# zama-ai/verifiable-fhe-paper

Hardware: AMD Instinct MI355X
Metric: vPBS proofs/sec at N=1024 (1/2/4/8 GPU); prover ms/proof vs CPU baseline (higher is better)
Workload: dtype u64; 1 GPU; N=1024 vPBS as IVC chain (BASELINE config 2; verified_pbs ivc_based_vpbs.rs:159-386) via vpbs_ivc_prove_pbs; step = 1 chained proof of the cyclic circuit (2^16 rows) per chain; chains_per_gpu=8, parallelism=replicas, witness=host

## Files before the change

bindings/rust/vpbs_sys.rs:

```rust
#![allow(non_camel_case_types, dead_code)]
use std::os::raw::{c_char, c_long, c_void};

pub const VPBS_POW_ANY: u64 = u64::MAX;
pub const VPBS_UNUSED_SELECTOR: u32 = 0xFFFF_FFFF;

#[repr(C)] pub struct VpbsCtx { _private: [u8; 0] }
#[repr(C)] pub struct VpbsBatch { _private: [u8; 0] }
#[repr(C)] pub struct VpbsWitnessPlan { _private: [u8; 0] }
#[repr(C)] pub struct VpbsWitnessState { _private: [u8; 0] }
#[repr(C)] pub struct VpbsWitnessDevice { _private: [u8; 0] }
#[repr(C)] pub struct VpbsWitnessChecker { _private: [u8; 0] }
#[repr(C)] pub struct VpbsProofVerifier { _private: [u8; 0] }
#[repr(C)] pub struct VpbsIvc { _private: [u8; 0] }
#[repr(C)] pub struct VpbsPbsVerifier { _private: [u8; 0] }
#[repr(C)] pub struct VpbsRingVerifier { _private: [u8; 0] }
#[repr(C)] pub struct VpbsBootstrapper { _private: [u8; 0] }
#[repr(C)] pub struct VpbsKeyring { _private: [u8; 0] }
#[repr(C)] pub struct VpbsPbsProver { _private: [u8; 0] }
#[repr(C)] pub struct VpbsRingProver { _private: [u8; 0] }
#[repr(C)] pub struct VpbsProgram { _private: [u8; 0] }

pub const VPBS_OK: i32 = 0;
pub const VPBS_ERR_INVALID: i32 = -1;
pub const VPBS_ERR_DEVICE: i32 = -2;
// ... 414 lines not shown
    pub fn vpbs_verify_step(in_: *const VpbsVerifyInputs, caps: *const u64, openings: *const u64, fri: *const u64) -> i32;
    pub fn vpbs_proof_verifier_create(ctx: *mut VpbsCtx, circuit: *const VpbsVerifyInputs, max_batch: usize, max_public_inputs: usize, out: *mut *mut VpbsProofVerifier, err: *mut c_char, err_len: usize) -> i32;
    pub fn vpbs_proof_verifier_run(v: *mut VpbsProofVerifier, bytes: *const u8, offsets: *const usize, count: usize, verdicts: *mut u8, reasons: *mut u8) -> c_long;
    pub fn vpbs_proof_verifier_free(v: *mut VpbsProofVerifier);
    pub fn vpbs_ivc_create(ctx: *mut VpbsCtx, cyclic: *const VpbsIvcCircuit, dummy: *const VpbsIvcCircuit, n: u32, k: u32, ggsw_len: usize, comm: *const VpbsComm, out: *mut *mut VpbsIvc, err: *mut c_char, err_len: usize) -> i32;
    pub fn vpbs_ivc_free(ivc: *mut VpbsIvc);
    pub fn vpbs_ivc_set_device_witness(ivc: *mut VpbsIvc, ell: u32, logb: u32, batch: u32, late_on_device: i32) -> i32;
    pub fn vpbs_ivc_set_check_witness(ivc: *mut VpbsIvc, on: i32) -> i32;
    pub fn vpbs_ivc_witness_checks(ivc: *const VpbsIvc, out: *mut u64) -> i32;
    pub fn vpbs_ivc_set_step_callback(ivc: *mut VpbsIvc, fn_: Option<VpbsIvcStepFn>, user: *mut c_void) -> i32;
    pub fn vpbs_ivc_last_error(ivc: *const VpbsIvc) -> *const c_char;
    pub fn vpbs_ivc_verifier_data(ivc: *const VpbsIvc, cyclic_vk: *mut u64, dummy_vk: *mut u64) -> i32;
    pub fn vpbs_ivc_prove_pbs(ivc: *mut VpbsIvc, testv: *const u64, ct: *const u64, bsk: *const u64, ksk: *const u64, n_lwe: u32, steps: u32, proof_out: *mut u8, capacity: usize, timing: *mut VpbsIvcTiming, err: *mut c_char, err_len: usize) -> c_long;
    pub fn vpbs_ivc_set_checkpoint(ivc: *mut VpbsIvc, every: u32, fn_: Option<VpbsIvcCheckpointFn>, user: *mut c_void) -> i32;
    pub fn vpbs_ivc_resume_pbs(ivc: *mut VpbsIvc, testv: *const u64, ct: *const u64, bsk: *const u64, ksk: *const u64, n_lwe: u32, checkpoint: *const u8, len: usize, steps: u32, proof_out: *mut u8, capacity: usize, timing: *mut VpbsIvcTiming, err: *mut c_char, err_len: usize) -> c_long;
    pub fn vpbs_verify_pbs(in_: *const VpbsVerifyPbsInputs, proof_bytes: *const u8, len: usize, why: *mut c_char, why_len: usize) -> i32;
    pub fn vpbs_verify_pbs_prefix(in_: *const VpbsVerifyPbsInputs, bytes: *const u8, len: usize, steps_done: *mut u32, why: *mut c_char, why_len: usize) -> i32;
    pub fn vpbs_pbs_reason_text(reason: i32) -> *const c_char;
    pub fn vpbs_pbs_key_hash(bsk: *const u64, ksk: *const u64, n_lwe: u32, ggsw_len: usize, out: *mut u64) -> i32;
    pub fn vpbs_pbs_verifier_create(ctx: *mut VpbsCtx, shape: *const VpbsVerifyPbsInputs, key_hash: *const u64, max_batch: usize, out: *mut *mut VpbsPbsVerifier, err: *mut c_char, err_len: usize) -> i32;
    pub fn vpbs_pbs_verifier_run(v: *mut VpbsPbsVerifier, bytes: *const u8, offsets: *const usize, count: usize, testv: *const u64, testv_per_proof: i32, ct: *const u64, out_ct: *const u64, verdicts: *mut u8, reasons: *mut u8, proof_reasons: *mut u8) -> c_long;
    pub fn vpbs_pbs_verifier_free(v: *mut VpbsPbsVerifier);
    pub fn vpbs_ring_verifier_create(ctx: *mut VpbsCtx, shape: *const VpbsVerifyPbsInputs, max_keys: u32, max_batch: usize, out: *mut *mut VpbsRingVerifier, err: *mut c_char, err_len: usize) -> i32;
    pub fn vpbs_ring_verifier_set_key(v: *mut VpbsRingVerifier, slot: u32, key_hash: *const u64) -> i32;
    pub fn vpbs_ring_verifier_clear_key(v: *mut VpbsRingVerifier, slot: u32) -> i32;
    pub fn vpbs_ring_verifier_count(v: *mut VpbsRingVerifier) -> c_long;
    pub fn vpbs_ring_verifier_run(v: *mut VpbsRingVerifier, bytes: *const u8, offsets: *const usize, count: usize, key_of: *const u32, testvs: *const u64, n_testv: usize, testv_of: *const u32, ct: *const u64, out_ct: *const u64, verdicts: *mut u8, reasons: *mut u8, proof_reasons: *mut u8, err: *mut c_char, err_len: usize) -> c_long;
    pub fn vpbs_ring_verifier_free(v: *mut VpbsRingVerifier);
    pub fn vpbs_k_poseidon_batch(ctx: *mut VpbsCtx, states: *mut u64, n: usize) -> i32;
    pub fn vpbs_k_hash_rows(ctx: *mut VpbsCtx, rows: *const u64, n: usize, len: u32, out: *mut u64) -> i32;
    pub fn vpbs_k_intt(ctx: *mut VpbsCtx, values: *const u64, ncols: u32, log_n: u32, coeffs_out: *mut u64) -> i32;
    pub fn vpbs_k_coset_lde(ctx: *mut VpbsCtx, coeffs: *const u64, ncols: u32, log_n: u32, rate_bits: u32, shift: u64, out: *mut u64) -> i32;
    pub fn vpbs_k_merkle_cap(ctx: *mut VpbsCtx, leaves: *const u64, n_leaves: usize, leaf_len: u32, cap_height: u32, cap_out: *mut u64) -> i32;
    pub fn vpbs_k_negacyclic_ntt(ctx: *mut VpbsCtx, data: *mut u64, batch: u32, log_n: u32, inverse: i32) -> i32;
    pub fn vpbs_k_poseidon_host(states: *mut u64, n: usize) -> i32;
    pub fn vpbs_k_clock_probe(ctx: *mut VpbsCtx, mhz_out: *mut f64) -> i32;
    pub fn vpbs_ntt_params(log_n: u32, roots: *mut u64, invroots: *mut u64, ninv: *mut u64) -> i32;
    pub fn vpbs_blind_rotate_step(ctx: *mut VpbsCtx, params: *const VpbsTfheParams, batch: u32, acc_in: *const u64, masks: *const u64, ggsw: *const u64, ggsw_per_instance: i32, first_step: i32, last_step: i32, acc_out: *mut u64, on_device: i32) -> i32;
    pub fn vpbs_pbs_accumulator_chain(ctx: *mut VpbsCtx, params: *const VpbsTfheParams, n: u32, acc_init: *const u64, lwe_ct: *const u64, bsk: *const u64, ksk: *const u64, accs_out: *mut u64) -> i32;
    pub fn vpbs_keygen(ctx: *mut VpbsCtx, params: *const VpbsKeygenParams, s_lwe: *mut u64, s_glwe: *mut u64, s_to: *mut u64, bsk: *mut u64, ksk: *mut u64, keys_on_device: i32) -> i32;
    pub fn vpbs_lwe_encrypt(params: *const VpbsKeygenParams, s_lwe: *const u64, message: u64, nonce: u64, ct: *mut u64) -> i32;
    pub fn vpbs_testv(log_n: u32, p: u32, testv: *mut u64, delta: *mut u64) -> i32;
    pub fn vpbs_glwe_decrypt(ctx: *mut VpbsCtx, log_n: u32, k: u32, s: *const u64, ct: *const u64, m_out: *mut u64) -> i32;
    pub fn vpbs_bootstrapper_create(ctx: *mut VpbsCtx, params: *const VpbsTfheParams, n_lwe: u32, bsk: *const u64, ksk: *const u64, keys_on_device: i32, max_batch: usize, out: *mut *mut VpbsBootstrapper, err: *mut c_char, err_len: usize) -> i32;
    pub fn vpbs_bootstrapper_run(b: *mut VpbsBootstrapper, cts: *const u64, count: usize, testv: *const u64, testv_per_ct: i32, out_ct: *mut u64, lwe_out: *mut u64, accs_out: *mut u64, on_device: i32) -> c_long;
    pub fn vpbs_bootstrapper_run_from(b: *mut VpbsBootstrapper, cts: *const u64, count: usize, start: *const u32, acc_in: *const u64, testv: *const u64, testv_per_ct: i32, out_ct: *mut u64, lwe_out: *mut u64, accs_out: *mut u64, on_device: i32) -> c_long;
    pub fn vpbs_bootstrapper_free(b: *mut VpbsBootstrapper);
    pub fn vpbs_lwe_extract(ctx: *mut VpbsCtx, log_n: u32, k: u32, n_lwe: u32, glwe: *const u64, count: usize, lwe_out: *mut u64, on_device: i32) -> i32;
    pub fn vpbs_lwe_decrypt(s_lwe: *const u64, ct: *const u64, n_lwe: u32, m_out: *mut u64) -> i32;
    pub fn vpbs_keyring_create(ctx: *mut VpbsCtx, params: *const VpbsTfheParams, n_lwe: u32, max_keys: usize, max_batch: usize, out: *mut *mut VpbsKeyring, err: *mut c_char, err_len: usize) -> i32;
    pub fn vpbs_keyring_add(ring: *mut VpbsKeyring, bsk: *const u64, ksk: *const u64, keys_on_device: i32, slot: *mut u32) -> i32;
    pub fn vpbs_keyring_remove(ring: *mut VpbsKeyring, slot: u32) -> i32;
    pub fn vpbs_keyring_count(ring: *mut VpbsKeyring) -> usize;
    pub fn vpbs_keyring_run(ring: *mut VpbsKeyring, cts: *const u64, count: usize, key_of: *const u32, testv: *const u64, testv_per_ct: i32, out_ct: *mut u64, lwe_out: *mut u64, accs_out: *mut u64, on_device: i32) -> c_long;
    pub fn vpbs_keyring_run_from(ring: *mut VpbsKeyring, cts: *const u64, count: usize, key_of: *const u32, start: *const u32, acc_in: *const u64, testv: *const u64, testv_per_ct: i32, out_ct: *mut u64, lwe_out: *mut u64, accs_out: *mut u64, on_device: i32) -> c_long;
    pub fn vpbs_keyring_free(ring: *mut VpbsKeyring);
    pub fn vpbs_lwe_encrypt_batch(ctx: *mut VpbsCtx, params: *const VpbsKeygenParams, s_lwe: *const u64, key_on_device: i32, messages: *const u64, count: usize, nonce0: u64, cts_out: *mut u64, on_device: i32) -> i32;
    pub fn vpbs_lut_testv(log_n: u32, p: u32, table: *const u64, delta: u64, testv: *mut u64) -> i32;
    pub fn vpbs_lwe_decode_batch(ctx: *mut VpbsCtx, s_lwe: *const u64, key_on_device: i32, cts: *const u64, count: usize, n_lwe: u32, delta: u64, modulus: u64, expected: *const u64, phase_out: *mut u64, msg_out: *mut u64, err_out: *mut u64, stats: *mut VpbsNoiseStats, on_device: i32) -> i32;
    pub fn vpbs_pbs_prover_create(device_ordinal: i32, cyclic: *const VpbsIvcCircuit, dummy: *const VpbsIvcCircuit, params: *const VpbsTfheParams, n_lwe: u32, bsk: *const u64, ksk: *const u64, keys_on_device: i32, chains: u32, witness_batch: u32, out: *mut *mut VpbsPbsProver, err: *mut c_char, err_len: usize) -> i32;
    pub fn vpbs_pbs_prover_run(p: *mut VpbsPbsProver, cts: *const u64, count: usize, testv: *const u64, testv_per_ct: i32, steps: u32, out_ct: *mut u64, lwe_out: *mut u64, proof_fn: Option<VpbsPbsProofFn>, user: *mut c_void, err: *mut c_char, err_len: usize) -> c_long;
    pub fn vpbs_pbs_prover_resume(p: *mut VpbsPbsProver, cts: *const u64, count: usize, testv: *const u64, testv_per_ct: i32, checkpoints: *const *const u8, lens: *const usize, steps: u32, out_ct: *mut u64, lwe_out: *mut u64, proof_fn: Option<VpbsPbsProofFn>, user: *mut c_void, err: *mut c_char, err_len: usize) -> c_long;
    pub fn vpbs_pbs_prover_key_hash(p: *const VpbsPbsProver, out: *mut u64) -> i32;
    pub fn vpbs_pbs_prover_verifier_data(p: *const VpbsPbsProver, cyclic_vk: *mut u64, dummy_vk: *mut u64) -> i32;
    pub fn vpbs_pbs_prover_set_check_witness(p: *mut VpbsPbsProver, on: i32) -> i32;
    pub fn vpbs_pbs_prover_witness_checks(p: *const VpbsPbsProver, out: *mut u64) -> i32;
// ... 44 lines not shown
```

include/vpbs_prover.h:

```cpp
#ifndef VPBS_PROVER_H
#define VPBS_PROVER_H
#include <stddef.h>
#include <stdint.h>

#ifdef __cplusplus
extern "C" {
#endif

typedef struct vpbs_ctx vpbs_ctx;
typedef struct vpbs_batch vpbs_batch;

typedef enum {
    VPBS_OK = 0,
    VPBS_ERR_INVALID = -1,
    VPBS_ERR_DEVICE = -2,
    VPBS_ERR_OOM = -3,
    VPBS_ERR_POW = -4,
    VPBS_ERR_PEER = -5,
    VPBS_ERR_WITNESS = -6
} vpbs_status;

#define VPBS_POW_ANY UINT64_MAX

int vpbs_ctx_create(int device_ordinal, unsigned log_n_max, unsigned rate_bits, unsigned cap_height, vpbs_ctx** out);
// ... 382 lines not shown
} vpbs_pbs_reason;
const char* vpbs_pbs_reason_text(int reason);
int vpbs_pbs_key_hash(const uint64_t* bsk , const uint64_t* ksk , unsigned n_lwe, size_t ggsw_len,
                      uint64_t out[4]);
typedef struct vpbs_pbs_verifier vpbs_pbs_verifier;
int vpbs_pbs_verifier_create(vpbs_ctx* ctx, const vpbs_verify_pbs_inputs* shape, const uint64_t key_hash[4], size_t max_batch,
                             vpbs_pbs_verifier** out, char* err, size_t err_len);
long vpbs_pbs_verifier_run(vpbs_pbs_verifier* v, const uint8_t* bytes, const size_t* offsets , size_t count,
                           const uint64_t* testv , int testv_per_proof, const uint64_t* ct ,
                           const uint64_t* out_ct , uint8_t* verdicts , uint8_t* reasons ,
                           uint8_t* proof_reasons );
void vpbs_pbs_verifier_free(vpbs_pbs_verifier* v);

typedef struct vpbs_ring_verifier vpbs_ring_verifier;
int vpbs_ring_verifier_create(vpbs_ctx* ctx, const vpbs_verify_pbs_inputs* shape, unsigned max_keys, size_t max_batch, vpbs_ring_verifier** out,
                              char* err, size_t err_len);
int vpbs_ring_verifier_set_key(vpbs_ring_verifier* v, unsigned slot, const uint64_t key_hash[4]);
int vpbs_ring_verifier_clear_key(vpbs_ring_verifier* v, unsigned slot);
long vpbs_ring_verifier_count(vpbs_ring_verifier* v);
long vpbs_ring_verifier_run(vpbs_ring_verifier* v, const uint8_t* bytes, const size_t* offsets , size_t count,
                            const uint32_t* key_of , const uint64_t* testvs , size_t n_testv,
                            const uint32_t* testv_of , const uint64_t* ct ,
                            const uint64_t* out_ct , uint8_t* verdicts , uint8_t* reasons ,
                            uint8_t* proof_reasons , char* err, size_t err_len);
void vpbs_ring_verifier_free(vpbs_ring_verifier* v);

int vpbs_k_poseidon_batch(vpbs_ctx* ctx, uint64_t* states , size_t n);
int vpbs_k_hash_rows(vpbs_ctx* ctx, const uint64_t* rows , size_t n, unsigned len, uint64_t* out );
int vpbs_k_intt(vpbs_ctx* ctx, const uint64_t* values, unsigned ncols, unsigned log_n, uint64_t* coeffs_out);
int vpbs_k_coset_lde(vpbs_ctx* ctx, const uint64_t* coeffs, unsigned ncols, unsigned log_n, unsigned rate_bits,
                     uint64_t shift, uint64_t* out);
int vpbs_k_merkle_cap(vpbs_ctx* ctx, const uint64_t* leaves, size_t n_leaves, unsigned leaf_len, unsigned cap_height,
                      uint64_t* cap_out);
int vpbs_k_negacyclic_ntt(vpbs_ctx* ctx, uint64_t* data, unsigned batch, unsigned log_n, int inverse);
int vpbs_k_poseidon_host(uint64_t* states, size_t n);
int vpbs_k_clock_probe(vpbs_ctx* ctx, double* mhz_out);
int vpbs_ntt_params(unsigned log_n, uint64_t* roots, uint64_t* invroots, uint64_t* ninv);

typedef struct {
    unsigned log_N;
    unsigned K;
    unsigned ELL;
    unsigned LOGB;
} vpbs_tfhe_params;
int vpbs_blind_rotate_step(vpbs_ctx* ctx, const vpbs_tfhe_params* params, unsigned batch, const uint64_t* acc_in,
                           const uint64_t* masks, const uint64_t* ggsw, int ggsw_per_instance, int first_step, int last_step,
                           uint64_t* acc_out, int on_device);

int vpbs_pbs_accumulator_chain(vpbs_ctx* ctx, const vpbs_tfhe_params* params, unsigned n, const uint64_t* acc_init,
                               const uint64_t* lwe_ct, const uint64_t* bsk, const uint64_t* ksk, uint64_t* accs_out);

typedef struct {
    unsigned log_N, K, ELL, LOGB;
    unsigned n_lwe;
    uint64_t seed;
    double sigma_glwe, sigma_lwe;
} vpbs_keygen_params;
int vpbs_keygen(vpbs_ctx* ctx, const vpbs_keygen_params* params, uint64_t* s_lwe, uint64_t* s_glwe, uint64_t* s_to, uint64_t* bsk,
                uint64_t* ksk, int keys_on_device);
int vpbs_lwe_encrypt(const vpbs_keygen_params* params, const uint64_t* s_lwe, uint64_t message, uint64_t nonce, uint64_t* ct);
int vpbs_testv(unsigned log_N, unsigned p, uint64_t* testv, uint64_t* delta);
int vpbs_glwe_decrypt(vpbs_ctx* ctx, unsigned log_N, unsigned K, const uint64_t* s, const uint64_t* ct, uint64_t* m_out);

typedef struct vpbs_bootstrapper vpbs_bootstrapper;
int vpbs_bootstrapper_create(vpbs_ctx* ctx, const vpbs_tfhe_params* params, unsigned n_lwe, const uint64_t* bsk, const uint64_t* ksk,
                             int keys_on_device, size_t max_batch, vpbs_bootstrapper** out, char* err, size_t err_len);
// ... 151 lines not shown
```

verifiable-fhe-paper_amd/api.py:

```python
import ctypes as C
import json
import math
import os
import subprocess
import weakref
from fractions import Fraction

import numpy as np

PKG_DIR = os.path.dirname(os.path.abspath(__file__))
LIB_PATH = os.path.join(PKG_DIR, "libvpbs_hip.so")
P = 0xFFFFFFFF00000001
POW_ANY = 0xFFFFFFFFFFFFFFFF
U64P = C.POINTER(C.c_uint64)
U32P = C.POINTER(C.c_uint32)


class VpbsError(RuntimeError):
    pass


ERR_WITNESS = -6


# ... 326 lines not shown
    "vpbs_ring_prover_keyring": (_vp, [_vp]),
    "vpbs_ring_prover_context": (_vp, [_vp]),
    "vpbs_ring_prover_run": (C.c_long, [_vp, U64P, _sz, _vp, U64P, _i, _ui, U64P, U64P, PBS_PROOF_FN, _vp, C.c_char_p, _sz]),
    "vpbs_ring_prover_resume": (C.c_long, [_vp, U64P, _sz, _vp, U64P, _i, _vp, _vp, _ui, U64P, U64P, PBS_PROOF_FN, _vp, C.c_char_p, _sz]),
    "vpbs_ring_prover_verifier_data": (_i, [_vp, U64P, U64P]),
    "vpbs_ring_prover_set_check_witness": (_i, [_vp, _i]),
    "vpbs_ring_prover_witness_checks": (_i, [_vp, U64P]),
    "vpbs_ring_prover_set_checkpoint": (_i, [_vp, _ui, PBS_CHECKPOINT_FN, _vp]),
    "vpbs_ring_prover_last_run": (_i, [_vp, C.POINTER(PbsRunStatsC)]),
    "vpbs_ring_prover_free": (None, [_vp]),
    "vpbs_program_create": (_i, [_vp, C.POINTER(ProgramDescC), C.POINTER(_vp), C.c_char_p, _sz]),
    "vpbs_program_levels": (C.c_long, [_vp, C.POINTER(_ui)]),
    "vpbs_program_run": (C.c_long, [_vp, _vp, _vp, _vp, _vp, _vp, _vp, _i]),
    "vpbs_program_run_batch": (C.c_long, [_vp, _vp, _vp, _sz, _vp, _vp, _vp, _vp, _vp, _i]),
    "vpbs_program_prove": (C.c_long, [_vp, _vp, U64P, U64P, _ui, U64P, U64P, PBS_PROOF_FN, _vp, C.c_char_p, _sz]),
    "vpbs_program_prove_batch": (C.c_long, [_vp, _vp, U64P, _sz, _vp, U64P, _ui, U64P, U64P, PBS_PROOF_FN, _vp, C.c_char_p, _sz]),
    "vpbs_program_verify": (C.c_long, [_vp, _vp, U64P, U64P, U64P, C.POINTER(C.c_uint8), C.POINTER(_sz), C.POINTER(C.c_uint8),
                                       C.POINTER(C.c_uint8), C.POINTER(C.c_uint8)]),
    "vpbs_program_verify_batch": (C.c_long, [_vp, _vp, U64P, _sz, _vp, U64P, U64P, C.POINTER(C.c_uint8), C.POINTER(_sz), C.POINTER(C.c_uint8),
                                             C.POINTER(C.c_uint8), C.POINTER(C.c_uint8), C.c_char_p, _sz]),
    "vpbs_program_free": (None, [_vp]),
    "vpbs_program_create_multi": (_i, [_vp, C.POINTER(ProgramDescC), C.POINTER(_ui), C.POINTER(_ui), C.POINTER(_vp), C.c_char_p, _sz]),
    "vpbs_program_wires": (C.c_long, [_vp, C.POINTER(_ui)]),
    "vpbs_lwe_snap": (_i, [_vp, _ui, _ui, _vp, _sz, _vp, _i]),
    "vpbs_lwe_extract_at": (_i, [_vp, _ui, _ui, _ui, _vp, _sz, _vp, _vp, _sz, _vp, _i]),
    "vpbs_lut_testv_multi": (_i, [_ui, _ui, _ui, U64P, _u64, U64P]),
    "vpbs_lwe_extract": (_i, [_vp, _ui, _ui, _ui, _vp, _sz, _vp, _i]),
    "vpbs_lwe_decrypt": (_i, [U64P, U64P, _ui, U64P]),
    "vpbs_lwe_encrypt_batch": (_i, [_vp, C.POINTER(KeygenParamsC), _vp, _i, _vp, _sz, _u64, _vp, _i]),
    "vpbs_lut_testv": (_i, [_ui, _ui, U64P, _u64, U64P]),
    "vpbs_lwe_decode_batch": (_i, [_vp, _vp, _i, _vp, _sz, _ui, _u64, _u64, _vp, _vp, _vp, _vp, C.POINTER(NoiseStatsC), _i]),
    "vpbs_k_poseidon_batch": (_i, [_vp, U64P, _sz]),
    "vpbs_k_hash_rows": (_i, [_vp, U64P, _sz, _ui, U64P]),
    "vpbs_k_intt": (_i, [_vp, U64P, _ui, _ui, U64P]),
    "vpbs_k_coset_lde": (_i, [_vp, U64P, _ui, _ui, _ui, _u64, U64P]),
    "vpbs_k_merkle_cap": (_i, [_vp, U64P, _sz, _ui, _ui, U64P]),
    "vpbs_k_negacyclic_ntt": (_i, [_vp, U64P, _ui, _ui, _i]),
    "vpbs_ntt_params": (_i, [_ui, U64P, U64P, U64P]),
    "vpbs_timing_enable": (_i, [_vp, _i]),
    "vpbs_timing_report": (_i, [_vp, C.c_char_p, _sz]),
    "vpbs_timing_shader_clock": (_i, [_vp, C.POINTER(C.c_double), C.POINTER(_ui)]),
}

INTERNAL_SIGNATURES = {
    "vpbs_test_ivc_preset_matrix": (_i, [_sz, _sz, _sz, _sz, _ui, _ui, _ui, U64P, U64P, U64P, U64P, U64P, U64P, U64P, U64P]),
    "vpbs_test_pbs_prover_preset_matrix": (_i, [_vp, U64P, U64P, _ui, _ui, U64P]),
    "vpbs_test_pbs_prover_preset_words": (_sz, [_vp]),
    "vpbs_test_pbs_prover_dummy_proof": (_i, [_vp, U64P]),
}

_lib = None


def build_library(force=False):
    args = ["make", "-C", os.path.join(PKG_DIR, "csrc"), "-j4"]
    if force:
        subprocess.check_call(args + ["clean"], stdout=subprocess.DEVNULL)
    subprocess.check_call(args, stdout=subprocess.DEVNULL)
    return LIB_PATH


def lib():
    global _lib
    if _lib is None:
        if not os.path.exists(LIB_PATH):
            raise VpbsError("libvpbs_hip.so is missing: run __graft_entry__.build() (make -C verifiable-fhe-paper_amd/csrc). "
# ... 2475 lines not shown
        self._check(lib().vpbs_k_clock_probe(self.h, C.byref(out)))
        return out.value

    def upload_bg(self, d_dst, host, words):
        if lib().vpbs_device_upload_bg(self.h, C.c_void_p(int(d_dst)), C.c_void_p(int(host)), int(words)):
            raise VpbsError("vpbs_device_upload_bg failed")

    def upload_rows(self, d_dst, host, n_cols, n, row_lo, row_hi):
        self._check(lib().vpbs_device_upload_rows(self.h, C.c_void_p(int(d_dst)), C.c_void_p(int(host)), n_cols, n, row_lo, row_hi))

    def scatter(self, d_dst, d_positions, host_values, count, d_stage):
        self._check(lib().vpbs_device_scatter(self.h, C.c_void_p(int(d_dst)), C.c_void_p(int(d_positions)), C.c_void_p(int(host_values)), count,
                                              C.c_void_p(int(d_stage))))

    def glwe_decrypt(self, s, ct):
        ct = _u64(ct)
        K, N = ct.shape
        s = np.ascontiguousarray(_u64(s)[:K - 1])
        out = np.zeros(N, np.uint64)
        self._check(lib().vpbs_glwe_decrypt(self.h, N.bit_length() - 1, K, _ptr(s), _ptr(ct), _ptr(out)))
        return out

    def poseidon_batch(self, states):
        s = _u64(states).copy()
        self._check(lib().vpbs_k_poseidon_batch(self.h, _ptr(s), s.shape[0]))
        return s

    def hash_rows(self, rows):
        r = _u64(rows)
        out = np.zeros((r.shape[0], 4), np.uint64)
        self._check(lib().vpbs_k_hash_rows(self.h, _ptr(r), r.shape[0], r.shape[1], _ptr(out)))
        return out

    def intt(self, values):
        v = _u64(values)
        out = np.zeros_like(v)
        self._check(lib().vpbs_k_intt(self.h, _ptr(v), v.shape[0], v.shape[1].bit_length() - 1, _ptr(out)))
        return out

    def coset_lde(self, coeffs, rate_bits=3, shift=7):
        c = _u64(coeffs)
        out = np.zeros((c.shape[0], c.shape[1] << rate_bits), np.uint64)
        self._check(lib().vpbs_k_coset_lde(self.h, _ptr(c), c.shape[0], c.shape[1].bit_length() - 1, rate_bits, shift, _ptr(out)))
        return out

    def merkle_cap(self, leaves, cap_height):
        l = _u64(leaves)
        out = np.zeros((1 << cap_height, 4), np.uint64)
        self._check(lib().vpbs_k_merkle_cap(self.h, _ptr(l), l.shape[0], l.shape[1], cap_height, _ptr(out)))
        return out

    def negacyclic_ntt(self, data, inverse=False):
        d = _u64(data).copy()
        self._check(lib().vpbs_k_negacyclic_ntt(self.h, _ptr(d), d.shape[0], d.shape[1].bit_length() - 1, 1 if inverse else 0))
        return d

    def timing_enable(self, on=1):
        self._check(lib().vpbs_timing_enable(self.h, int(on)))

    def timing_report(self):
        buf = C.create_string_buffer(8192)
        self._check(lib().vpbs_timing_report(self.h, buf, 8192))
        return json.loads(buf.value.decode())
```

verifiable-fhe-paper_amd/csrc/api.hip:

```cpp
#include <atomic>
#include <sys/prctl.h>
#include <time.h>
#include <chrono>
#include <condition_variable>
#include <cstdlib>
#include <cstring>
#include <memory>
#include <mutex>
#include <unordered_map>

#include "context.h"
#include "poseidon.h"
#include "host/poseidon_x8.h"

using vpbs::DeviceError;
using vpbs::u64;

void* vpbs_ctx::alloc_bytes(size_t bytes) {
    if (bytes == 0) bytes = 8;
    bytes = (bytes + 255) & ~(size_t)255;
    auto it = free_blocks.find(bytes);
    if (it != free_blocks.end()) {
        void* p = it->second;
        free_blocks.erase(it);
// ... 848 lines not shown
        u64* d_out = c->alloc_words(a.record_words);
        auto* d_args = static_cast<vpbs::OpenArgs*>(c->alloc_bytes(sizeof a));
        VPBS_HIP(hipMemcpyAsync(d_args, &a, sizeof a, hipMemcpyHostToDevice, c->stream));
        vpbs::launch_open_queries(c->stream, d_args, 1, 1, d_out);
        std::vector<u64> rec(a.record_words);
        VPBS_HIP(hipMemcpyAsync(rec.data(), d_out, sizeof(u64) * a.record_words, hipMemcpyDeviceToHost, c->stream));
        VPBS_HIP(vpbs::stream_sync(c->stream));
        std::memcpy(leaf_out, rec.data(), sizeof(u64) * b->ncols);
        std::memcpy(siblings_out, rec.data() + b->ncols, sizeof(u64) * 4 * t.n_siblings);
        c->release(d_out);
        c->release(d_args);
    });
}

int vpbs_k_poseidon_batch(vpbs_ctx* c, uint64_t* states, size_t n) {
    if (!c || !states) return VPBS_ERR_INVALID;
    return guarded(c, [&] {
        DevTemp d(c, states, 12 * n);
        vpbs::launch_permute_batch(c->stream, d.p, n);
        VPBS_HIP(hipMemcpyAsync(states, d.p, sizeof(u64) * 12 * n, hipMemcpyDeviceToHost, c->stream));
        VPBS_HIP(vpbs::stream_sync(c->stream));
    });
}
int vpbs_k_hash_rows(vpbs_ctx* c, const uint64_t* rows, size_t n, unsigned len, uint64_t* out) {
    if (!c || !rows || !out || len == 0) return VPBS_ERR_INVALID;
    return guarded(c, [&] {
        DevTemp d(c, rows, n * len);
        DevTemp o(c, nullptr, 4 * n);
        vpbs::launch_hash_rows(c->stream, d.p, n, len, o.p);
        VPBS_HIP(hipMemcpyAsync(out, o.p, sizeof(u64) * 4 * n, hipMemcpyDeviceToHost, c->stream));
        VPBS_HIP(vpbs::stream_sync(c->stream));
    });
}
int vpbs_k_intt(vpbs_ctx* c, const uint64_t* values, unsigned ncols, unsigned log_n, uint64_t* coeffs_out) {
    if (!c || !values || !coeffs_out) return VPBS_ERR_INVALID;
    return guarded(c, [&] {
        const size_t words = (size_t)ncols << log_n;
        DevTemp in(c, values, words), out(c, nullptr, words), scratch(c, nullptr, words);
        vpbs::launch_intt(c->stream, in.p, out.p, scratch.p, c->roots(log_n, true), ncols, log_n);
        VPBS_HIP(hipMemcpyAsync(coeffs_out, out.p, sizeof(u64) * words, hipMemcpyDeviceToHost, c->stream));
        VPBS_HIP(vpbs::stream_sync(c->stream));
    });
}
int vpbs_k_coset_lde(vpbs_ctx* c, const uint64_t* coeffs, unsigned ncols, unsigned log_n, unsigned rate_bits, uint64_t shift,
                     uint64_t* out_host) {
    if (!c || !coeffs || !out_host) return VPBS_ERR_INVALID;
    return guarded(c, [&] {
        const size_t words = (size_t)ncols << log_n;
        DevTemp in(c, coeffs, words), out(c, nullptr, words << rate_bits);
        vpbs::launch_coset_lde(c->stream, in.p, out.p, c->roots(log_n, false), c->lde_table(log_n, rate_bits, shift), ncols, log_n,
                               rate_bits);
        VPBS_HIP(hipMemcpyAsync(out_host, out.p, sizeof(u64) * (words << rate_bits), hipMemcpyDeviceToHost, c->stream));
        VPBS_HIP(vpbs::stream_sync(c->stream));
    });
}
int vpbs_k_merkle_cap(vpbs_ctx* c, const uint64_t* leaves, size_t n_leaves, unsigned leaf_len, unsigned cap_height, uint64_t* cap_out) {
    if (!c || !leaves || !cap_out || leaf_len == 0) return VPBS_ERR_INVALID;
    return guarded(c, [&] {
        std::vector<size_t> off;
        const size_t words = vpbs::merkle_layout(n_leaves, cap_height, off);
        DevTemp in(c, leaves, n_leaves * leaf_len), dig(c, nullptr, words);
        if (leaf_len <= 4) {
            std::vector<u64> padded(4 * n_leaves, 0);
            for (size_t i = 0; i < n_leaves; ++i)
                for (unsigned k = 0; k < leaf_len; ++k) padded[4 * i + k] = leaves[i * leaf_len + k];
            VPBS_HIP(hipMemcpyAsync(dig.p, padded.data(), sizeof(u64) * 4 * n_leaves, hipMemcpyHostToDevice, c->stream));
// ... 340 lines not shown
```

verifiable-fhe-paper_amd/csrc/hash.hip:

```cpp
#include <cstdlib>

#include <algorithm>
#include "kernels.h"
#include "poseidon.h"

namespace vpbs {
namespace {
constexpr unsigned THREADS = 256;

template <bool SAMPLE>
__global__ void __launch_bounds__(THREADS)
leaf_hash_kernel(const u64* __restrict__ lde, unsigned ncols, size_t n_leaves, size_t col_stride, u64* __restrict__ digests,
                 u64* __restrict__ clock_sample) {
    const size_t j = blockIdx.x * (size_t)THREADS + threadIdx.x;
    if (j >= n_leaves) return;
    const bool sample = SAMPLE && clock_sample != nullptr && blockIdx.x == gridDim.x / 2 && threadIdx.x == 0;
    u64 c0 = 0, r0 = 0;
    if (sample) {
        r0 = __builtin_amdgcn_s_memrealtime();
        c0 = __builtin_amdgcn_s_memtime();
    }
    u64 s[12];
#pragma unroll
    for (int i = 0; i < 12; ++i) s[i] = 0;
    if (ncols <= 4) {
#pragma unroll
        for (int k = 0; k < 4; ++k)
            if ((unsigned)k < ncols) s[k] = lde[k * col_stride + j];
    } else {
        u64 nxt[8];
#pragma unroll
        for (int k = 0; k < 8; ++k) nxt[k] = (unsigned)k < ncols ? lde[(size_t)k * col_stride + j] : 0;
        for (unsigned c0 = 0; c0 < ncols; c0 += 8) {
#pragma unroll
            for (int k = 0; k < 8; ++k)
                if (c0 + k < ncols) s[k] = nxt[k];
            if (c0 + 8 < ncols) {
#pragma unroll
                for (int k = 0; k < 8; ++k)
                    if (c0 + 8 + k < ncols) nxt[k] = lde[(size_t)(c0 + 8 + k) * col_stride + j];
            }
            poseidon::permute_residues(s);
        }
#pragma unroll
        for (int k = 0; k < 4; ++k) s[k] = gl::canon(s[k]);
    }
    ulonglong2* d = reinterpret_cast<ulonglong2*>(digests + 4 * j);
    d[0] = make_ulonglong2(s[0], s[1]);
    d[1] = make_ulonglong2(s[2], s[3]);
    if (sample) {
        clock_sample[0] = __builtin_amdgcn_s_memtime() - c0;
        clock_sample[1] = __builtin_amdgcn_s_memrealtime() - r0;
    }
}

__global__ void __launch_bounds__(THREADS)
fri_leaf_hash_kernel(const u64* __restrict__ v0, const u64* __restrict__ v1, size_t n_leaves, unsigned arity_bits,
                     u64* __restrict__ digests) {
    const size_t l = blockIdx.x * (size_t)THREADS + threadIdx.x;
    if (l >= n_leaves) return;
    const unsigned arity = 1u << arity_bits;
    const size_t base = l << arity_bits;
    u64 s[12];
#pragma unroll
    for (int i = 0; i < 12; ++i) s[i] = 0;
    if (2 * arity <= 4) {
        for (unsigned m = 0; m < arity; ++m) { s[2 * m] = v0[base + m]; s[2 * m + 1] = v1[base + m]; }
    } else {
        for (unsigned m0 = 0; m0 < arity; m0 += 4) {
#pragma unroll
            for (int k = 0; k < 4; ++k)
                if (m0 + k < arity) { s[2 * k] = v0[base + m0 + k]; s[2 * k + 1] = v1[base + m0 + k]; }
            poseidon::permute_residues(s);
        }
#pragma unroll
        for (int k = 0; k < 4; ++k) s[k] = gl::canon(s[k]);
    }
    ulonglong2* d = reinterpret_cast<ulonglong2*>(digests + 4 * l);
    d[0] = make_ulonglong2(s[0], s[1]);
    d[1] = make_ulonglong2(s[2], s[3]);
}

__global__ void __launch_bounds__(THREADS)
merkle_level_kernel(const u64* __restrict__ children, u64* __restrict__ parents, size_t n_parents) {
    const size_t i = blockIdx.x * (size_t)THREADS + threadIdx.x;
    if (i >= n_parents) return;
    const ulonglong2* c = reinterpret_cast<const ulonglong2*>(children + 8 * i);
    const ulonglong2 a = c[0], b = c[1], e = c[2], f = c[3];
    u64 s[12] = {a.x, a.y, b.x, b.y, e.x, e.y, f.x, f.y, 0, 0, 0, 0};
    poseidon::permute_residues(s);
#pragma unroll
    for (int k = 0; k < 4; ++k) s[k] = gl::canon(s[k]);
    ulonglong2* d = reinterpret_cast<ulonglong2*>(parents + 4 * i);
    d[0] = make_ulonglong2(s[0], s[1]);
    d[1] = make_ulonglong2(s[2], s[3]);
}

__global__ void __launch_bounds__(THREADS)
merkle_level_wide_kernel(const u64* __restrict__ children, u64* __restrict__ parents, size_t n_parents) {
    __shared__ u64 lds[(THREADS / poseidon::WIDE_LANES) * poseidon::WIDE_LDS_WORDS];
    const unsigned l = threadIdx.x & 15, g = threadIdx.x >> 4;
    const size_t i = blockIdx.x * (size_t)(THREADS / 16) + g;
    const bool live = i < n_parents;
    u64 x = (live && l < 8) ? children[8 * i + l] : 0;
    x = poseidon::permute_wide(x, lds + g * poseidon::WIDE_LDS_WORDS, l);
    if (live && l < 4) parents[4 * i + l] = x;
}

constexpr unsigned CLIMB_THREADS = 512, CLIMB_MAX_LEVELS = 6;
struct ClimbArgs {
    const u64* children;
// ... 46 lines not shown

__global__ void __launch_bounds__(THREADS) permute_batch_kernel(u64* states, size_t n) {
    const size_t i = blockIdx.x * (size_t)THREADS + threadIdx.x;
    if (i >= n) return;
    u64 s[12];
#pragma unroll
    for (int k = 0; k < 12; ++k) s[k] = states[12 * i + k];
    poseidon::permute(s);
#pragma unroll
    for (int k = 0; k < 12; ++k) states[12 * i + k] = s[k];
}

__global__ void __launch_bounds__(THREADS)
hash_rows_kernel(const u64* __restrict__ rows, size_t n, unsigned len, u64* __restrict__ out) {
    const size_t i = blockIdx.x * (size_t)THREADS + threadIdx.x;
    if (i >= n) return;
    const u64* row = rows + i * len;
    u64 s[12];
#pragma unroll
    for (int k = 0; k < 12; ++k) s[k] = 0;
    for (unsigned c0 = 0; c0 < len; c0 += 8) {
#pragma unroll
        for (int k = 0; k < 8; ++k)
            if (c0 + k < len) s[k] = row[c0 + k];
        poseidon::permute_residues(s);
    }
#pragma unroll
    for (int k = 0; k < 4; ++k) out[4 * i + k] = gl::canon(s[k]);
}

struct PowState {
    u64 s[12];
};

__global__ void __launch_bounds__(THREADS)
pow_search_kernel(PowState st, unsigned pos, unsigned pow_bits, u64 start, u64 count, u64 stride, unsigned long long* result) {
    const u64 i = blockIdx.x * (u64)THREADS + threadIdx.x;
    if (i >= stride) return;
    for (u64 off = i; off < count; off += stride) {
        const u64 cand = start + off;
        if (__atomic_load_n(result, __ATOMIC_RELAXED) < cand) return;
        u64 s[12];
#pragma unroll
        for (int k = 0; k < 12; ++k) s[k] = (unsigned)k == pos ? cand : st.s[k];
        poseidon::permute_residues(s);
        if (pow_bits == 0 || (gl::canon(s[7]) >> (64 - pow_bits)) == 0) {
            atomicMin(result, (unsigned long long)cand);
            return;
        }
    }
}
}

void launch_leaf_hash(hipStream_t s, const u64* lde, unsigned ncols, size_t n_leaves, size_t col_stride, u64* digests, u64* clock_sample) {
    if (clock_sample)
        hipLaunchKernelGGL(leaf_hash_kernel<true>, dim3((n_leaves + THREADS - 1) / THREADS), dim3(THREADS), 0, s, lde, ncols, n_leaves,
                           col_stride, digests, clock_sample);
    else
        hipLaunchKernelGGL(leaf_hash_kernel<false>, dim3((n_leaves + THREADS - 1) / THREADS), dim3(THREADS), 0, s, lde, ncols, n_leaves,
                           col_stride, digests, clock_sample);
}
Tuning Tuning::from_env() {
    Tuning t;
    if (const char* e = getenv("VPBS_WIDE_THRESHOLD")) t.wide_threshold = t.fri_leaf_wide_threshold = (size_t)strtoull(e, nullptr, 10);
    if (const char* e = getenv("VPBS_FRI_LEAF_WIDE_THRESHOLD")) t.fri_leaf_wide_threshold = (size_t)strtoull(e, nullptr, 10);
    if (const char* e = getenv("VPBS_MERKLE_CLIMB")) t.merkle_climb = atoi(e) != 0;
    if (const char* e = getenv("VPBS_GATES_FUSED")) t.gates_fused = atoi(e) != 0;
    if (const char* e = getenv("VPBS_GATE_ITEMS")) t.gate_items = (unsigned)std::max(1, atoi(e));
    if (const char* e = getenv("VPBS_GATES_TILE")) t.gates_tile = atoi(e) != 0;
    return t;
}

void launch_fri_leaf_hash(hipStream_t s, const Tuning& tune, const u64* v0, const u64* v1, size_t n_leaves, unsigned arity_bits, u64* digests) {
    if (n_leaves <= tune.fri_leaf_wide_threshold && (2u << arity_bits) > 4) {
        hipLaunchKernelGGL(fri_leaf_hash_wide_kernel, dim3((unsigned)((n_leaves * 16 + THREADS - 1) / THREADS)), dim3(THREADS), 0, s, v0,
                           v1, n_leaves, arity_bits, digests);
        return;
    }
    hipLaunchKernelGGL(fri_leaf_hash_kernel, dim3((n_leaves + THREADS - 1) / THREADS), dim3(THREADS), 0, s, v0, v1, n_leaves,
                       arity_bits, digests);
}
void launch_merkle_level(hipStream_t s, const Tuning& tune, const u64* children, u64* parents, size_t n_parents) {
    if (n_parents <= tune.wide_threshold) {
        hipLaunchKernelGGL(merkle_level_wide_kernel, dim3((unsigned)((n_parents * 16 + THREADS - 1) / THREADS)), dim3(THREADS), 0, s,
                           children, parents, n_parents);
        return;
    }
    hipLaunchKernelGGL(merkle_level_kernel, dim3((n_parents + THREADS - 1) / THREADS), dim3(THREADS), 0, s, children, parents,
                       n_parents);
}
void launch_merkle_tree(hipStream_t s, const Tuning& tune, u64* digests, const size_t* level_off, unsigned n_levels, size_t n_leaves) {
    unsigned k = 1;
    for (; k < n_levels && (n_leaves >> k) > tune.wide_threshold; ++k)
        launch_merkle_level(s, tune, digests + level_off[k - 1], digests + level_off[k], n_leaves >> k);
    const bool fused = tune.merkle_climb;
    while (k < n_levels) {
        const size_t n_children = n_leaves >> (k - 1);
        unsigned levels = std::min(CLIMB_MAX_LEVELS, n_levels - k);
        if (!fused || levels < 2) {
            launch_merkle_level(s, tune, digests + level_off[k - 1], digests + level_off[k], n_leaves >> k);
            ++k;
            continue;
        }
        ClimbArgs a{};
        a.children = digests + level_off[k - 1];
        a.levels = levels;
        for (unsigned j = 0; j < levels; ++j) a.out[j] = digests + level_off[k + j];
        hipLaunchKernelGGL(merkle_climb_wide_kernel, dim3((unsigned)(n_children >> levels)), dim3(CLIMB_THREADS), 0, s, a);
        k += levels;
    }
}
void launch_permute_batch(hipStream_t s, u64* states, size_t n) {
    hipLaunchKernelGGL(permute_batch_kernel, dim3((n + THREADS - 1) / THREADS), dim3(THREADS), 0, s, states, n);
}
void launch_hash_rows(hipStream_t s, const u64* rows, size_t n, unsigned len, u64* out) {
    hipLaunchKernelGGL(hash_rows_kernel, dim3((n + THREADS - 1) / THREADS), dim3(THREADS), 0, s, rows, n, len, out);
}
void launch_pow_search(hipStream_t s, const Tuning& tune, const u64* state12_host, unsigned pos, unsigned pow_bits, u64 start, u64 count,
                       u64* d_result) {
    PowState st;
    for (int k = 0; k < 12; ++k) st.s[k] = state12_host[k];
    const bool shared_gpu = tune.wide_threshold < ((size_t)1 << 14);
    const u64 stride = shared_gpu ? std::min<u64>(count, (u64)1 << 15) : count;
    hipLaunchKernelGGL(pow_search_kernel, dim3((unsigned)((stride + THREADS - 1) / THREADS)), dim3(THREADS), 0, s, st, pos, pow_bits,
                       start, count, stride, reinterpret_cast<unsigned long long*>(d_result));
}
}
```

Baseline: 0.2021 vPBS proofs/s.

## Stage leaf-hash column loads via LDS and re-read kernel args to cut VGPRs

The Merkle leaf-hash kernel now prefetches the next 8 columns with global_load_lds into per-wave LDS planes instead of holding them in registers. The FRI leaf-hash and PoW search kernels take a single argument struct and re-read scalar fields through the kernarg pointer, using readfirstlane and asm barriers so values stay in SGPRs. The goal is lower vector-register pressure around the Poseidon permutation and higher occupancy. It adds LDS use, explicit waitcnt synchronisation and fragile inline-asm tricks, plus new test entry points for the three kernels.

```diff
diff --git a/bindings/rust/vpbs_sys.rs b/bindings/rust/vpbs_sys.rs
--- a/bindings/rust/vpbs_sys.rs
+++ b/bindings/rust/vpbs_sys.rs
@@ -470,6 +470,9 @@
     pub fn vpbs_k_intt(ctx: *mut VpbsCtx, values: *const u64, ncols: u32, log_n: u32, coeffs_out: *mut u64) -> i32;
     pub fn vpbs_k_coset_lde(ctx: *mut VpbsCtx, coeffs: *const u64, ncols: u32, log_n: u32, rate_bits: u32, shift: u64, out: *mut u64) -> i32;
     pub fn vpbs_k_merkle_cap(ctx: *mut VpbsCtx, leaves: *const u64, n_leaves: usize, leaf_len: u32, cap_height: u32, cap_out: *mut u64) -> i32;
+    pub fn vpbs_k_leaf_hash(ctx: *mut VpbsCtx, lde: *const u64, ncols: u32, n_leaves: usize, col_stride: usize, out: *mut u64) -> i32;
+    pub fn vpbs_k_fri_leaf_hash(ctx: *mut VpbsCtx, v0: *const u64, v1: *const u64, n_leaves: usize, arity_bits: u32, out: *mut u64) -> i32;
+    pub fn vpbs_k_pow_search(ctx: *mut VpbsCtx, state12: *const u64, pos: u32, pow_bits: u32, start: u64, count: u64, nonce_out: *mut u64) -> i32;
     pub fn vpbs_k_negacyclic_ntt(ctx: *mut VpbsCtx, data: *mut u64, batch: u32, log_n: u32, inverse: i32) -> i32;
     pub fn vpbs_k_poseidon_host(states: *mut u64, n: usize) -> i32;
     pub fn vpbs_k_clock_probe(ctx: *mut VpbsCtx, mhz_out: *mut f64) -> i32;
diff --git a/include/vpbs_prover.h b/include/vpbs_prover.h
--- a/include/vpbs_prover.h
+++ b/include/vpbs_prover.h
@@ -438,6 +438,12 @@
                      uint64_t shift, uint64_t* out);
 int vpbs_k_merkle_cap(vpbs_ctx* ctx, const uint64_t* leaves, size_t n_leaves, unsigned leaf_len, unsigned cap_height,
                       uint64_t* cap_out);
+int vpbs_k_leaf_hash(vpbs_ctx* ctx, const uint64_t* lde , unsigned ncols, size_t n_leaves, size_t col_stride,
+                     uint64_t* out );
+int vpbs_k_fri_leaf_hash(vpbs_ctx* ctx, const uint64_t* v0 , const uint64_t* v1, size_t n_leaves,
+                         unsigned arity_bits, uint64_t* out );
+int vpbs_k_pow_search(vpbs_ctx* ctx, const uint64_t state12[12], unsigned pos, unsigned pow_bits, uint64_t start, uint64_t count,
+                      uint64_t* nonce_out);
 int vpbs_k_negacyclic_ntt(vpbs_ctx* ctx, uint64_t* data, unsigned batch, unsigned log_n, int inverse);
 int vpbs_k_poseidon_host(uint64_t* states, size_t n);
 int vpbs_k_clock_probe(vpbs_ctx* ctx, double* mhz_out);
diff --git a/verifiable-fhe-paper_amd/api.py b/verifiable-fhe-paper_amd/api.py
--- a/verifiable-fhe-paper_amd/api.py
+++ b/verifiable-fhe-paper_amd/api.py
@@ -382,6 +382,9 @@
     "vpbs_lwe_decode_batch": (_i, [_vp, _vp, _i, _vp, _sz, _ui, _u64, _u64, _vp, _vp, _vp, _vp, C.POINTER(NoiseStatsC), _i]),
     "vpbs_k_poseidon_batch": (_i, [_vp, U64P, _sz]),
     "vpbs_k_hash_rows": (_i, [_vp, U64P, _sz, _ui, U64P]),
+    "vpbs_k_leaf_hash": (_i, [_vp, U64P, _ui, _sz, _sz, U64P]),
+    "vpbs_k_fri_leaf_hash": (_i, [_vp, U64P, U64P, _sz, _ui, U64P]),
+    "vpbs_k_pow_search": (_i, [_vp, U64P, _ui, _ui, _u64, _u64, U64P]),
     "vpbs_k_intt": (_i, [_vp, U64P, _ui, _ui, U64P]),
     "vpbs_k_coset_lde": (_i, [_vp, U64P, _ui, _ui, _ui, _u64, U64P]),
     "vpbs_k_merkle_cap": (_i, [_vp, U64P, _sz, _ui, _ui, U64P]),
@@ -2923,6 +2926,26 @@
         self._check(lib().vpbs_k_hash_rows(self.h, _ptr(r), r.shape[0], r.shape[1], _ptr(out)))
         return out
 
+    def leaf_hash(self, lde, n_leaves=None):
+        d = _u64(lde)
+        n = d.shape[1] if n_leaves is None else int(n_leaves)
+        out = np.zeros((n, 4), np.uint64)
+        self._check(lib().vpbs_k_leaf_hash(self.h, _ptr(d), d.shape[0], n, d.shape[1], _ptr(out)))
+        return out
+
+    def fri_leaf_hash(self, v0, v1, arity_bits):
+        a, b = _u64(v0), _u64(v1)
+        n = a.shape[0] >> arity_bits
+        out = np.zeros((n, 4), np.uint64)
+        self._check(lib().vpbs_k_fri_leaf_hash(self.h, _ptr(a), _ptr(b), n, arity_bits, _ptr(out)))
+        return out
+
+    def pow_search(self, state12, pos, pow_bits, start, count):
+        st = _u64(state12)
+        out = np.zeros(1, np.uint64)
+        self._check(lib().vpbs_k_pow_search(self.h, _ptr(st), pos, pow_bits, start, count, _ptr(out)))
+        return None if int(out[0]) == (1 << 64) - 1 else int(out[0])
+
     def intt(self, values):
         v = _u64(values)
         out = np.zeros_like(v)
diff --git a/verifiable-fhe-paper_amd/csrc/api.hip b/verifiable-fhe-paper_amd/csrc/api.hip
--- a/verifiable-fhe-paper_amd/csrc/api.hip
+++ b/verifiable-fhe-paper_amd/csrc/api.hip
@@ -904,6 +904,39 @@
         VPBS_HIP(vpbs::stream_sync(c->stream));
     });
 }
+int vpbs_k_leaf_hash(vpbs_ctx* c, const uint64_t* lde, unsigned ncols, size_t n_leaves, size_t col_stride, uint64_t* out) {
+    if (!c || !lde || !out || ncols == 0 || n_leaves == 0 || col_stride < n_leaves) return VPBS_ERR_INVALID;
+    return guarded(c, [&] {
+        DevTemp d(c, lde, (size_t)ncols * col_stride);
+        DevTemp o(c, nullptr, 4 * n_leaves);
+        vpbs::launch_leaf_hash(c->stream, d.p, ncols, n_leaves, col_stride, o.p);
+        VPBS_HIP(hipMemcpyAsync(out, o.p, sizeof(u64) * 4 * n_leaves, hipMemcpyDeviceToHost, c->stream));
+        VPBS_HIP(vpbs::stream_sync(c->stream));
+    });
+}
+int vpbs_k_fri_leaf_hash(vpbs_ctx* c, const uint64_t* v0, const uint64_t* v1, size_t n_leaves, unsigned arity_bits, uint64_t* out) {
+    if (!c || !v0 || !v1 || !out || n_leaves == 0 || arity_bits > 8) return VPBS_ERR_INVALID;
+    return guarded(c, [&] {
+        DevTemp a(c, v0, n_leaves << arity_bits), b(c, v1, n_leaves << arity_bits);
+        DevTemp o(c, nullptr, 4 * n_leaves);
+        vpbs::Tuning lane_form = c->tune;
+        lane_form.fri_leaf_wide_threshold = 0;
+        vpbs::launch_fri_leaf_hash(c->stream, lane_form, a.p, b.p, n_leaves, arity_bits, o.p);
+        VPBS_HIP(hipMemcpyAsync(out, o.p, sizeof(u64) * 4 * n_leaves, hipMemcpyDeviceToHost, c->stream));
+        VPBS_HIP(vpbs::stream_sync(c->stream));
+    });
+}
+int vpbs_k_pow_search(vpbs_ctx* c, const uint64_t state12[12], unsigned pos, unsigned pow_bits, uint64_t start, uint64_t count,
+                      uint64_t* nonce_out) {
+    if (!c || !state12 || !nonce_out || pos >= 12 || pow_bits > 63 || count == 0) return VPBS_ERR_INVALID;
+    return guarded(c, [&] {
+        DevTemp r(c, nullptr, 1);
+        VPBS_HIP(hipMemsetAsync(r.p, 0xFF, sizeof(u64), c->stream));
+        vpbs::launch_pow_search(c->stream, c->tune, state12, pos, pow_bits, start, count, r.p);
+        VPBS_HIP(hipMemcpyAsync(nonce_out, r.p, sizeof(u64), hipMemcpyDeviceToHost, c->stream));
+        VPBS_HIP(vpbs::stream_sync(c->stream));
+    });
+}
 int vpbs_k_intt(vpbs_ctx* c, const uint64_t* values, unsigned ncols, unsigned log_n, uint64_t* coeffs_out) {
     if (!c || !values || !coeffs_out) return VPBS_ERR_INVALID;
     return guarded(c, [&] {
diff --git a/verifiable-fhe-paper_amd/csrc/hash.hip b/verifiable-fhe-paper_amd/csrc/hash.hip
--- a/verifiable-fhe-paper_amd/csrc/hash.hip
+++ b/verifiable-fhe-paper_amd/csrc/hash.hip
@@ -8,12 +8,52 @@
 namespace {
 constexpr unsigned THREADS = 256;
 
+constexpr unsigned STAGE_PLANE = 64 * sizeof(unsigned), STAGE_PER_WAVE = 8 * 2 * STAGE_PLANE;
+
+__device__ __forceinline__ unsigned uniform(unsigned x) { return (unsigned)__builtin_amdgcn_readfirstlane(x); }
+
+struct Staging {
+    const u64* rows;
+    size_t col_stride;
+    unsigned at;
+    unsigned mine;
+    char* wave_lds;
+    __device__ __forceinline__ Staging(const u64* lde, size_t n_leaves, size_t stride, char* stage) {
+        unsigned t = threadIdx.x, wg = blockIdx.x, n_lo = (unsigned)n_leaves, n_hi = (unsigned)(n_leaves >> 32);
+        unsigned stride_lo = (unsigned)stride, stride_hi = (unsigned)(stride >> 32);
+        asm volatile("" : "+v"(t), "+s"(wg), "+s"(n_lo), "+s"(n_hi), "+s"(stride_lo), "+s"(stride_hi));
+        wg = uniform(wg);
+        n_lo = uniform(n_lo);
+        n_hi = uniform(n_hi);
+        rows = lde + wg * (size_t)THREADS;
+        col_stride = (size_t)uniform(stride_hi) << 32 | uniform(stride_lo);
+        const unsigned last = wg < (unsigned)(((size_t)n_hi << 32 | n_lo) / THREADS) ? THREADS - 1 : n_lo % THREADS - 1;
+        at = std::min(t, last) * (unsigned)sizeof(u64);
+        mine = t / 64 * STAGE_PER_WAVE + t % 64 * (unsigned)sizeof(unsigned);
+        wave_lds = stage + uniform(mine);
+    }
+    __device__ __forceinline__ void load(unsigned c, unsigned ncols) const {
+        typedef __attribute__((address_space(1))) const void* gptr_t;
+        typedef __attribute__((address_space(3))) void* lptr_t;
+#pragma unroll
+        for (int k = 0; k < 8; ++k)
+            if (c + k < ncols) {
+                unsigned a = at;
+                asm volatile("" : "+v"(a));
+                const char* src = reinterpret_cast<const char*>(rows + (size_t)(c + k) * col_stride) + a;
+                __builtin_amdgcn_global_load_lds((gptr_t)src, (lptr_t)(wave_lds + (2 * k) * STAGE_PLANE), 4, 0, 0);
+                __builtin_amdgcn_global_load_lds((gptr_t)src, (lptr_t)(wave_lds + (2 * k + 1) * STAGE_PLANE - 4), 4, 4, 0);
+            }
+    }
+};
+
 template <bool SAMPLE>
 __global__ void __launch_bounds__(THREADS)
 leaf_hash_kernel(const u64* __restrict__ lde, unsigned ncols, size_t n_leaves, size_t col_stride, u64* __restrict__ digests,
                  u64* __restrict__ clock_sample) {
-    const size_t j = blockIdx.x * (size_t)THREADS + threadIdx.x;
-    if (j >= n_leaves) return;
+    __shared__ char stage[(THREADS / 64) * STAGE_PER_WAVE];
+    const size_t first = blockIdx.x * (size_t)THREADS;
+    const u64* __restrict__ rows = lde + first;
     const bool sample = SAMPLE && clock_sample != nullptr && blockIdx.x == gridDim.x / 2 && threadIdx.x == 0;
     u64 c0 = 0, r0 = 0;
     if (sample) {
@@ -24,59 +64,89 @@
 #pragma unroll
     for (int i = 0; i < 12; ++i) s[i] = 0;
     if (ncols <= 4) {
+        const unsigned last = (unsigned)std::min<size_t>(n_leaves - 1 - first, THREADS - 1);
+        const unsigned t = std::min(threadIdx.x, last);
 #pragma unroll
         for (int k = 0; k < 4; ++k)
-            if ((unsigned)k < ncols) s[k] = lde[k * col_stride + j];
+            if ((unsigned)k < ncols) s[k] = rows[k * col_stride + t];
     } else {
-        u64 nxt[8];
-#pragma unroll
-        for (int k = 0; k < 8; ++k) nxt[k] = (unsigned)k < ncols ? lde[(size_t)k * col_stride + j] : 0;
+        Staging(lde, n_leaves, col_stride, stage).load(0, ncols);
         for (unsigned c0 = 0; c0 < ncols; c0 += 8) {
+            const Staging g(lde, n_leaves, col_stride, stage);
+            asm volatile("s_waitcnt vmcnt(0)" ::: "memory");
 #pragma unroll
             for (int k = 0; k < 8; ++k)
-                if (c0 + k < ncols) s[k] = nxt[k];
+                if (c0 + k < ncols) {
+                    const unsigned* w = reinterpret_cast<const unsigned*>(stage + g.mine + 2 * k * STAGE_PLANE);
+                    s[k] = (u64)w[STAGE_PLANE / sizeof(unsigned)] << 32 | w[0];
+                }
             if (c0 + 8 < ncols) {
-#pragma unroll
-                for (int k = 0; k < 8; ++k)
-                    if (c0 + 8 + k < ncols) nxt[k] = lde[(size_t)(c0 + 8 + k) * col_stride + j];
+                asm volatile("s_waitcnt lgkmcnt(0)" ::: "memory");
+                g.load(c0 + 8, ncols);
             }
             poseidon::permute_residues(s);
+            asm volatile("" : "+s"(c0));
         }
 #pragma unroll
         for (int k = 0; k < 4; ++k) s[k] = gl::canon(s[k]);
     }
-    ulonglong2* d = reinterpret_cast<ulonglong2*>(digests + 4 * j);
-    d[0] = make_ulonglong2(s[0], s[1]);
-    d[1] = make_ulonglong2(s[2], s[3]);
+    const size_t j = first + threadIdx.x;
+    if (j < n_leaves) {
+        ulonglong2* d = reinterpret_cast<ulonglong2*>(digests + 4 * j);
+        d[0] = make_ulonglong2(s[0], s[1]);
+        d[1] = make_ulonglong2(s[2], s[3]);
+    }
     if (sample) {
         clock_sample[0] = __builtin_amdgcn_s_memtime() - c0;
         clock_sample[1] = __builtin_amdgcn_s_memrealtime() - r0;
     }
 }
 
-__global__ void __launch_bounds__(THREADS)
-fri_leaf_hash_kernel(const u64* __restrict__ v0, const u64* __restrict__ v1, size_t n_leaves, unsigned arity_bits,
-                     u64* __restrict__ digests) {
+template <typename T>
+__device__ __forceinline__ const __attribute__((address_space(4))) T* kernel_args() {
+    uintptr_t args = (uintptr_t)__builtin_amdgcn_kernarg_segment_ptr();
+    unsigned lo = (unsigned)args, hi = (unsigned)(args >> 32);
+    asm volatile("" : "+s"(lo), "+s"(hi));
+    return (const __attribute__((address_space(4))) T*)((uintptr_t)uniform(hi) << 32 | uniform(lo));
+}
+
+struct FriLeafArgs {
+    const u64 *v0, *v1;
+    size_t n_leaves;
+    unsigned arity_bits;
+    u64* digests;
+};
+__global__ void __launch_bounds__(THREADS) fri_leaf_hash_kernel(FriLeafArgs a) {
     const size_t l = blockIdx.x * (size_t)THREADS + threadIdx.x;
-    if (l >= n_leaves) return;
-    const unsigned arity = 1u << arity_bits;
-    const size_t base = l << arity_bits;
+    if (l >= a.n_leaves) return;
     u64 s[12];
 #pragma unroll
     for (int i = 0; i < 12; ++i) s[i] = 0;
-    if (2 * arity <= 4) {
-        for (unsigned m = 0; m < arity; ++m) { s[2 * m] = v0[base + m]; s[2 * m + 1] = v1[base + m]; }
+    if ((2u << a.arity_bits) <= 4) {
+        const size_t base = l << a.arity_bits;
+        for (unsigned m = 0; m < (1u << a.arity_bits); ++m) { s[2 * m] = a.v0[base + m]; s[2 * m + 1] = a.v1[base + m]; }
     } else {
-        for (unsigned m0 = 0; m0 < arity; m0 += 4) {
+        for (unsigned m0 = 0; m0 < (1u << a.arity_bits); m0 += 4) {
+            const auto* g = kernel_args<FriLeafArgs>();
+            unsigned t = threadIdx.x, wg = blockIdx.x;
+            asm volatile("" : "+v"(t), "+s"(wg));
+            const unsigned bits = g->arity_bits, arity = 1u << bits;
+            const size_t first = (((size_t)uniform(wg) * THREADS) << bits) + m0;
+            const unsigned lane_at = (t << bits) * (unsigned)sizeof(u64);
 #pragma unroll
             for (int k = 0; k < 4; ++k)
-                if (m0 + k < arity) { s[2 * k] = v0[base + m0 + k]; s[2 * k + 1] = v1[base + m0 + k]; }
+                if (m0 + k < arity) {
+                    unsigned at = lane_at;
+                    asm volatile("" : "+v"(at));
+                    s[2 * k] = *reinterpret_cast<const u64*>(reinterpret_cast<const char*>(g->v0 + first + k) + at);
+                    s[2 * k + 1] = *reinterpret_cast<const u64*>(reinterpret_cast<const char*>(g->v1 + first + k) + at);
+                }
             poseidon::permute_residues(s);
         }
 #pragma unroll
         for (int k = 0; k < 4; ++k) s[k] = gl::canon(s[k]);
     }
-    ulonglong2* d = reinterpret_cast<ulonglong2*>(digests + 4 * l);
+    ulonglong2* d = reinterpret_cast<ulonglong2*>(a.digests + 4 * l);
     d[0] = make_ulonglong2(s[0], s[1]);
     d[1] = make_ulonglong2(s[2], s[3]);
 }
@@ -189,22 +259,37 @@
 struct PowState {
     u64 s[12];
 };
-
-__global__ void __launch_bounds__(THREADS)
-pow_search_kernel(PowState st, unsigned pos, unsigned pow_bits, u64 start, u64 count, u64 stride, unsigned long long* result) {
-    const u64 i = blockIdx.x * (u64)THREADS + threadIdx.x;
-    if (i >= stride) return;
-    for (u64 off = i; off < count; off += stride) {
-        const u64 cand = start + off;
-        if (__atomic_load_n(result, __ATOMIC_RELAXED) < cand) return;
+struct PowArgs {
+    PowState st;
+    unsigned pos, pow_bits;
+    u64 start, count, stride;
+    unsigned long long* result;
+};
+
+__global__ void __launch_bounds__(THREADS) pow_search_kernel(PowArgs) {
+    u64 off = blockIdx.x * (u64)THREADS + threadIdx.x;
+    bool go;
+    {
+        const auto* a = kernel_args<PowArgs>();
+        go = off < a->stride && off < a->count && __atomic_load_n(a->result, __ATOMIC_RELAXED) >= a->start + off;
+    }
+    while (go) {
         u64 s[12];
-#pragma unroll
-        for (int k = 0; k < 12; ++k) s[k] = (unsigned)k == pos ? cand : st.s[k];
+        {
+            const auto* a = kernel_args<PowArgs>();
+            const unsigned pos = a->pos;
+            const u64 cand = a->start + off;
+#pragma unroll
+            for (int k = 0; k < 12; ++k) s[k] = (unsigned)k == pos ? cand : a->st.s[k];
+        }
         poseidon::permute_residues(s);
-        if (pow_bits == 0 || (gl::canon(s[7]) >> (64 - pow_bits)) == 0) {
-            atomicMin(result, (unsigned long long)cand);
-            return;
-        }
+        const auto* a = kernel_args<PowArgs>();
+        const unsigned pow_bits = a->pow_bits;
+        const u64 cand = a->start + off;
+        const bool valid = pow_bits == 0 || (gl::canon(s[7]) >> (64 - pow_bits)) == 0;
+        if (valid) atomicMin(a->result, (unsigned long long)cand);
+        off += a->stride;
+        go = !valid & (off < a->count) & (__atomic_load_n(a->result, __ATOMIC_RELAXED) >= a->start + off);
     }
 }
 }
@@ -234,8 +319,8 @@
                            v1, n_leaves, arity_bits, digests);
         return;
     }
-    hipLaunchKernelGGL(fri_leaf_hash_kernel, dim3((n_leaves + THREADS - 1) / THREADS), dim3(THREADS), 0, s, v0, v1, n_leaves,
-                       arity_bits, digests);
+    hipLaunchKernelGGL(fri_leaf_hash_kernel, dim3((n_leaves + THREADS - 1) / THREADS), dim3(THREADS), 0, s,
+                       FriLeafArgs{v0, v1, n_leaves, arity_bits, digests});
 }
 void launch_merkle_level(hipStream_t s, const Tuning& tune, const u64* children, u64* parents, size_t n_parents) {
     if (n_parents <= tune.wide_threshold) {
@@ -275,11 +360,15 @@
 }
 void launch_pow_search(hipStream_t s, const Tuning& tune, const u64* state12_host, unsigned pos, unsigned pow_bits, u64 start, u64 count,
                        u64* d_result) {
-    PowState st;
-    for (int k = 0; k < 12; ++k) st.s[k] = state12_host[k];
+    PowArgs a;
+    for (int k = 0; k < 12; ++k) a.st.s[k] = state12_host[k];
+    a.pos = pos;
+    a.pow_bits = pow_bits;
+    a.start = start;
+    a.count = count;
+    a.result = reinterpret_cast<unsigned long long*>(d_result);
     const bool shared_gpu = tune.wide_threshold < ((size_t)1 << 14);
-    const u64 stride = shared_gpu ? std::min<u64>(count, (u64)1 << 15) : count;
-    hipLaunchKernelGGL(pow_search_kernel, dim3((unsigned)((stride + THREADS - 1) / THREADS)), dim3(THREADS), 0, s, st, pos, pow_bits,
-                       start, count, stride, reinterpret_cast<unsigned long long*>(d_result));
-}
-}
+    a.stride = shared_gpu ? std::min<u64>(count, (u64)1 << 15) : count;
+    hipLaunchKernelGGL(pow_search_kernel, dim3((unsigned)((a.stride + THREADS - 1) / THREADS)), dim3(THREADS), 0, s, a);
+}
+}
```

After: 0.2041 vPBS proofs/s, median of 6. 1.0% higher.
